# QuantumSavory/LDPCDecoders.jl

Measured on AMD Instinct MI355X. Metric: decoded syndromes/sec (batchdecode!, 50 iters) + achieved HBM GB/s fraction, higher is better.
Workload: dtype f64

## Files before the change

### ldpcdecoders.jl_amd/csrc/bp_kernels.hpp

```cpp
#pragma once
#include <hip/hip_runtime.h>
#include <stdint.h>

#include "team_layout.hpp"

namespace ldpc {

typedef unsigned long long u64;

#ifndef LDPC_MIN_WAVES
#define LDPC_MIN_WAVES 6
#endif
#ifndef LDPC_STM_SC1
#define LDPC_STM_SC1 0
#endif
#ifndef LDPC_NT
#define LDPC_NT 0
#endif
#ifndef LDPC_ROTATE
#define LDPC_ROTATE 1
#endif
#ifndef LDPC_PHASE_TICKS
#define LDPC_PHASE_TICKS 1
#endif
#ifndef LDPC_SLOT_PAD
#define LDPC_SLOT_PAD 1053184
#endif

template <int DC, int DV, int THREADS>
constexpr int min_waves_per_simd()
{
    constexpr int one_block = THREADS / 256;
#ifndef LDPC_MIN_WAVES_MID
#define LDPC_MIN_WAVES_MID 3
#endif
    int want = (DC <= 8 && DV <= 4) ? LDPC_MIN_WAVES : (DC <= 16 ? LDPC_MIN_WAVES_MID : 2);
    if (want < one_block) want = one_block;
    if (THREADS >= 1024 && want > 4) want = 4;
    return want;
}

#ifndef LDPC_LOADS_FIRST
#define LDPC_LOADS_FIRST 0
#endif
__device__ __forceinline__ void loads_first()
{
#if LDPC_LOADS_FIRST
    __builtin_amdgcn_sched_barrier(0);
#endif
}

__device__ __forceinline__ double ldm(const double *p)
{
#if LDPC_NT
    return __builtin_nontemporal_load(p);
#else
    return *p;
#endif
}
__device__ __forceinline__ void stm(double *p, double v)
{
#if LDPC_STM_SC1
    __hip_atomic_store(p, v, __ATOMIC_RELAXED, __HIP_MEMORY_SCOPE_AGENT);
#elif LDPC_NT
    __builtin_nontemporal_store(v, p);
#else
    *p = v;
#endif
}

struct BPCold {
    int *iters;
// ... 187 lines not shown
        out[k] = TF ? t : (1.0 - t) / (1.0 + t);
        S = S * a[k];
    }
#endif
}

template <int D, bool FIRST, bool TF = false>
__device__ __forceinline__ double check_update_exact(double *M, double sigma, double r, double S0 = 1.0)
{
    double a[D];
    if (FIRST) {
        const double a0 = 2.0 / (1.0 + r) - 1.0;
#pragma unroll
        for (int k = 0; k < D; ++k) a[k] = a0;
    } else {
        double m[D];
#pragma unroll
        for (int k = 0; k < D; ++k) m[k] = ldm(M + (size_t)k * kTile);
        check_factors<D>(m, a);
    }
    return check_finish_exact<D, TF>(M, a, sigma, S0);
}

template <int D, bool TF = false>
__device__ __forceinline__ void check_update_pair(double *M0, double *M1, double sigma0, double sigma1)
{
    double m0[D], m1[D];
#pragma unroll
    for (int k = 0; k < D; ++k) m0[k] = ldm(M0 + (size_t)k * kTile);
#pragma unroll
    for (int k = 0; k < D; ++k) m1[k] = ldm(M1 + (size_t)k * kTile);
    loads_first();
    double a[D];
    check_factors<D>(m0, a);
    check_finish_exact<D, TF>(M0, a, sigma0);
    check_factors<D>(m1, a);
    check_finish_exact<D, TF>(M1, a, sigma1);
}

template <bool FIRST>
__device__ __noinline__ void check_update_any(double *M, int deg, double sigma, double r)
{
    double S = 1.0;
    for (int k = deg - 1; k >= 0; --k) {
        double P = sigma;
        for (int q = 0; q < k; ++q) {
            const double m = FIRST ? r : M[(size_t)q * kTile];
            P = P * (2.0 / (1.0 + m) - 1.0);
        }
        const double mk = FIRST ? r : M[(size_t)k * kTile];
        const double ak = 2.0 / (1.0 + mk) - 1.0;
        const double t = P * S;
        M[(size_t)k * kTile] = (1.0 - t) / (1.0 + t);
        S = S * ak;
    }
// ... 180 lines not shown
    }
}

template <int DV>
__device__ __forceinline__ double bit_update(double *Mt, const int *__restrict__ pos, int deg, double r)
{
    if (deg == DV) return bit_update_exact<DV>(Mt, pos, r);
    if (deg == 0) return r;
    if (deg < DV) return bit_dispatch<1, DV - 1>(Mt, pos, deg, r);
    return bit_update_any(Mt, pos, deg, r);
}

__device__ __forceinline__ unsigned int defer_reserve(unsigned int *count, unsigned int cnt, unsigned int cap)
{
    unsigned int old = __hip_atomic_load(count, __ATOMIC_RELAXED, __HIP_MEMORY_SCOPE_AGENT);
    for (;;) {
        if (old + cnt > cap || old + cnt < old) return ~0u;
        const unsigned int prev = atomicCAS(count, old, old + cnt);
        if (prev == old) return old;
        old = prev;
    }
}

__device__ __forceinline__ void defer_copy_rows(const double *Mt, double *dst, bool mine, int nnz, int first, int step)
{
    int e = first;
    for (; e + 7 * step < nnz; e += 8 * step) {
        double v[8];
#pragma unroll
        for (int k = 0; k < 8; ++k) v[k] = Mt[(size_t)(e + k * step) * kTile];
        if (mine) {
#pragma unroll
            for (int k = 0; k < 8; ++k) dst[(size_t)(e + k * step) * kTile] = v[k];
        }
    }
    for (; e < nnz; e += step) {
        const double v = Mt[(size_t)e * kTile];
        if (mine) dst[(size_t)e * kTile] = v;
    }
}

template <int DC, int DV, bool WANT_LLR, int THREADS, bool SECOND>
__global__ void
__launch_bounds__(THREADS, (min_waves_per_simd<DC, DV, THREADS>()))
bp_tile_kernel(BPParams p, const int *__restrict__ row_ptr, const int *__restrict__ edge_bit,
               const int *__restrict__ col_ptr, const int *__restrict__ csc2csr,
               const u64 *__restrict__ synmask, const u64 *__restrict__ nevermask)
{
// ... 359 lines not shown
```

### ldpcdecoders.jl_amd/csrc/bp_team_kernels.hpp

```cpp
#pragma once
#include "bp_kernels.hpp"

#ifndef LDPC_TEAM_ROWS_WIDE
#define LDPC_TEAM_ROWS_WIDE 1
#endif
#ifndef LDPC_TEAM_TFORM
#define LDPC_TEAM_TFORM 1
#endif
#ifndef LDPC_TEAM_TEST_DIRECT
#define LDPC_TEAM_TEST_DIRECT 1
#endif
#ifndef LDPC_TEAM_SLEEP
#define LDPC_TEAM_SLEEP 16
#endif

namespace ldpc {


template <int DV>
struct TeamVRec {
    int pos[DV], lrow[DV], bit;
};
template <int DV>
__device__ __forceinline__ TeamVRec<DV> team_vrec_load(const int *__restrict__ vt)
// ... 203 lines not shown
                if ((polls & 31u) == 0u && wall_clock64() - t0 > (u64)ticks) {
                    bool dead = false;
                    while (c < (unsigned)G && !dead)
                        dead = __hip_atomic_compare_exchange_strong(word, &c, c | DEAD, __ATOMIC_RELAXED, __ATOMIC_RELAXED,
                                                                    __HIP_MEMORY_SCOPE_AGENT);
                    if (dead) __hip_atomic_store(fault, ticket | kTeamRollcallFailed, __ATOMIC_RELAXED, __HIP_MEMORY_SCOPE_SYSTEM);
                    if (dead || (c & DEAD)) { ok = 0; break; }
                }
            }
        }
        *sh_ok = ok;
    }
    __syncthreads();
    return *sh_ok != 0;
}

__device__ __forceinline__ int team_deal(unsigned int *counter, int lane)
{
    unsigned int t = 0;
    if (lane == 0) t = atomicAdd(counter, 1u);
    return __builtin_amdgcn_readfirstlane((int)t);
}

template <int D, bool FIRST, bool TF = false>
__device__ __forceinline__ void check_update_mixed(double *M, double *L, unsigned int mask, double sigma, double r)
{
    double *ptr[D];
    int nl = 0;
#pragma unroll
    for (int k = 0; k < D; ++k) {
        const bool in_lds = (mask >> k) & 1u;
        ptr[k] = in_lds ? L + (size_t)nl * kTile : M + (size_t)k * kTile;
        nl += in_lds ? 1 : 0;
    }
    double a[D], out[D];
    if (FIRST) {
        const double a0 = 2.0 / (1.0 + r) - 1.0;
#pragma unroll
        for (int k = 0; k < D; ++k) a[k] = a0;
    } else {
        double m[D];
#pragma unroll
        for (int k = 0; k < D; ++k) m[k] = *ptr[k];
        check_factors<D>(m, a);
    }
    check_compute_exact<D, TF>(a, sigma, out);
#pragma unroll
    for (int k = D - 1; k >= 0; --k) *ptr[k] = out[k];
}

template <int D, bool TF = false>
__device__ __forceinline__ double bit_update_mixed(double *Mt, double *L, const int (&pos)[D], const int (&lrow)[D], double r)
{
    double *ptr[D];
#pragma unroll
    for (int k = 0; k < D; ++k) {
        const bool in_lds = lrow[k] >= 0;
        ptr[k] = (in_lds ? L : Mt) + (size_t)(in_lds ? lrow[k] : pos[k]) * kTile;
    }
    double c[D], out[D];
#pragma unroll
    for (int k = 0; k < D; ++k) c[k] = *ptr[k];
    if (TF) check_to_odds<D>(c, c);
    const double F = bit_compute_exact<D>(c, r, out);
#pragma unroll
    for (int k = D - 1; k >= 0; --k) *ptr[k] = out[k];
    return F;
}

template <int D, bool FIRST, bool TF, class RGet, class RPut>
__device__ __forceinline__ void check_update_onchip(double *M, double *L, double *Ld, unsigned int mask, unsigned int rmask, int rbase,
                                                    double sigma, double r, RGet &&rget, RPut &&rput)
{
    double *ptr[D];
    int nl = 0;
#pragma unroll
    for (int k = 0; k < D; ++k) {
        const bool in_lds = (mask >> k) & 1u, in_reg = (rmask >> k) & 1u;
        ptr[k] = in_reg ? Ld : (in_lds ? L + (size_t)nl * kTile : M + (size_t)k * kTile);
        nl += in_lds ? 1 : 0;
    }
    double a[D], out[D];
    if (FIRST) {
        const double a0 = 2.0 / (1.0 + r) - 1.0;
#pragma unroll
        for (int k = 0; k < D; ++k) a[k] = a0;
    } else {
        double m[D];
#pragma unroll
        for (int k = 0; k < D; ++k) m[k] = *ptr[k];
#pragma unroll
        for (int k = 0; k < D; ++k)
            if ((rmask >> k) & 1u) m[k] = rget(rbase + __builtin_popcount(rmask & ((1u << k) - 1u)));
        check_factors<D>(m, a);
    }
    check_compute_exact<D, TF>(a, sigma, out);
#pragma unroll
    for (int k = D - 1; k >= 0; --k) *ptr[k] = out[k];
#pragma unroll
    for (int k = D - 1; k >= 0; --k) rput((rmask >> k) & 1u, rbase + __builtin_popcount(rmask & ((1u << k) - 1u)), out[k]);
}

template <int D, bool TF, class RGet, class RPut>
__device__ __forceinline__ double bit_update_onchip(double *Mt, double *L, double *Ld, const int (&pos)[D], const int (&loc)[D], double r,
                                                    RGet &&rget, RPut &&rput)
{
    double *ptr[D];
#pragma unroll
    for (int k = 0; k < D; ++k) {
        const bool in_lds = loc[k] >= 0;
        ptr[k] = loc[k] <= -2 ? Ld : (in_lds ? L : Mt) + (size_t)(in_lds ? loc[k] : pos[k]) * kTile;
    }
    double c[D], out[D];
#pragma unroll
    for (int k = 0; k < D; ++k) c[k] = *ptr[k];
#pragma unroll
    for (int k = 0; k < D; ++k)
        if (loc[k] <= -2) c[k] = rget(-2 - loc[k]);
    if (TF) check_to_odds<D>(c, c);
    const double F = bit_compute_exact<D>(c, r, out);
#pragma unroll
    for (int k = D - 1; k >= 0; --k) *ptr[k] = out[k];
#pragma unroll
    for (int k = D - 1; k >= 0; --k) rput(loc[k] <= -2, -2 - loc[k], out[k]);
    return F;
}

template <int D, bool FIRST, bool TF, class RGet, class RPut>
__device__ __forceinline__ void check_update_regs(int rbase, double sigma, double r, RGet &&rget, RPut &&rput)
{
    double a[D], out[D];
    if (FIRST) {
        const double a0 = 2.0 / (1.0 + r) - 1.0;
#pragma unroll
        for (int k = 0; k < D; ++k) a[k] = a0;
    } else {
        double m[D];
#pragma unroll
        for (int k = 0; k < D; ++k) m[k] = rget(rbase + k);
        check_factors<D>(m, a);
    }
    check_compute_exact<D, TF>(a, sigma, out);
#pragma unroll
    for (int k = D - 1; k >= 0; --k) rput(true, rbase + k, out[k]);
}

template <int D, bool TF, class RGet, class RPut>
__device__ __forceinline__ void bit_update_pair_first(double *Mt, double *L, const int (&pos0)[D], const int loc0, const int (&pos1)[D],
                                                      const int loc1, double r, RGet &&rget, RPut &&rput, double &T0, double &T1)
{
    double c0[D], c1[D], o0[D], o1[D];
    size_t at0[D], at1[D];
#pragma unroll
    for (int k = 0; k < D; ++k) { at0[k] = (size_t)pos0[k] * kTile; at1[k] = (size_t)pos1[k] * kTile; }
#pragma unroll
    for (int k = 1; k < D; ++k) c0[k] = ldm(Mt + at0[k]);
#pragma unroll
    for (int k = 1; k < D; ++k) c1[k] = ldm(Mt + at1[k]);
    if (loc0 == -1) c0[0] = ldm(Mt + at0[0]);
    else if (loc0 >= 0) c0[0] = L[(size_t)loc0 * kTile];
    else c0[0] = rget(-2 - loc0);
    if (loc1 == -1) c1[0] = ldm(Mt + at1[0]);
    else if (loc1 >= 0) c1[0] = L[(size_t)loc1 * kTile];
    else c1[0] = rget(-2 - loc1);
    loads_first();
    if (TF) { check_to_odds<D>(c0, c0); check_to_odds<D>(c1, c1); }
    T0 = bit_compute_exact<D>(c0, r, o0);
#pragma unroll
    for (int k = D - 1; k >= 1; --k) stm(Mt + at0[k], o0[k]);
    if (loc0 == -1) stm(Mt + at0[0], o0[0]);
    else if (loc0 >= 0) L[(size_t)loc0 * kTile] = o0[0];
    else rput(true, -2 - loc0, o0[0]);
    T1 = bit_compute_exact<D>(c1, r, o1);
#pragma unroll
    for (int k = D - 1; k >= 1; --k) stm(Mt + at1[k], o1[k]);
    if (loc1 == -1) stm(Mt + at1[0], o1[0]);
    else if (loc1 >= 0) L[(size_t)loc1 * kTile] = o1[0];
    else rput(true, -2 - loc1, o1[0]);
}

template <int D, int NB, bool TF, int KIND, class RGet, class RPut>
__device__ __forceinline__ void bit_update_multi_first(double *Mt, double *L, const int (&pos)[NB][D], const int (&loc)[NB], double r,
                                                       RGet &&rget, RPut &&rput, double (&T)[NB])
{
    double c[NB][D];
#pragma unroll
    for (int b = 0; b < NB; ++b) {
#pragma unroll
        for (int k = 1; k < D; ++k) c[b][k] = ldm(Mt + (size_t)pos[b][k] * kTile);
    }
#pragma unroll
    for (int b = 0; b < NB; ++b) {
        if (KIND == 1) c[b][0] = L[(size_t)loc[b] * kTile];
        else if (KIND == 2) c[b][0] = rget(-2 - loc[b]);
        else if (loc[b] == -1) c[b][0] = ldm(Mt + (size_t)pos[b][0] * kTile);
        else if (loc[b] >= 0) c[b][0] = L[(size_t)loc[b] * kTile];
        else c[b][0] = rget(-2 - loc[b]);
    }
    loads_first();
#pragma unroll
    for (int b = 0; b < NB; ++b) {
        if (TF) check_to_odds<D>(c[b], c[b]);
        double o[D];
        T[b] = bit_compute_exact<D>(c[b], r, o);
#pragma unroll
        for (int k = D - 1; k >= 1; --k) stm(Mt + (size_t)pos[b][k] * kTile, o[k]);
        if (KIND == 1) L[(size_t)loc[b] * kTile] = o[0];
        else if (KIND == 2) rput(true, -2 - loc[b], o[0]);
        else if (loc[b] == -1) stm(Mt + (size_t)pos[b][0] * kTile, o[0]);
        else if (loc[b] >= 0) L[(size_t)loc[b] * kTile] = o[0];
        else rput(true, -2 - loc[b], o[0]);
    }
}

template <int D, int DC, bool TF, class RPut>
__device__ __forceinline__ double bit_update_first(double *Mt, double *L, const double *first, const u64 *__restrict__ syn, int lane,
                                                   const int (&pos)[D], const int (&loc)[D], double r, RPut &&rput)
{
    double c[D], out[D];
#pragma unroll
    for (int k = 0; k < D; ++k) {
        const int i = pos[k] / DC, place = pos[k] - i * DC;
        const bool odd = (syn[i] >> lane) & 1ull;
        c[k] = first[(odd ? DC : 0) + place];
    }
    if (TF) check_to_odds<D>(c, c);
    const double F = bit_compute_exact<D>(c, r, out);
#pragma unroll
    for (int k = D - 1; k >= 0; --k) {
        if (loc[k] == -1) stm(Mt + (size_t)pos[k] * kTile, out[k]);
        else if (loc[k] >= 0) L[(size_t)loc[k] * kTile] = out[k];
        else rput(true, -2 - loc[k], out[k]);
    }
    return F;
}

#ifndef LDPC_TEAM_TEST_SPREAD
#define LDPC_TEAM_TEST_SPREAD 1
#endif
#ifndef LDPC_TEAM_FAULT_BLOCKS
#ifdef LDPC_EXPERIMENTS
#define LDPC_TEAM_FAULT_BLOCKS 1
#else
#define LDPC_TEAM_FAULT_BLOCKS 0
#endif
#endif
#ifndef LDPC_TEAM_LIKELY
#define LDPC_TEAM_LIKELY 1
#endif
#ifndef LDPC_TEAM_FUSE_FIRST
#define LDPC_TEAM_FUSE_FIRST 1
#endif
#ifndef LDPC_TEAM_FUSE_DC_MAX
#define LDPC_TEAM_FUSE_DC_MAX 10
// ... 52 lines not shown
__global__ void
__launch_bounds__(THREADS, (team_min_waves_per_simd<DC, DV, THREADS, LROWS || IRR>()))
bp_team_kernel(BPParams p, TeamParams tp, const int *__restrict__ row_ptr, const int *__restrict__ edge_bit,
               const int *__restrict__ col_ptr, const int *__restrict__ csc2csr,
               const u64 *__restrict__ synmask, const u64 *__restrict__ nevermask)
{
    static_assert(!(LROWS && RESUMED), "packed tiles are decoded where they lie, all rows in global memory");
    static_assert(RR == 0 || (LROWS && RR == kTeamRegRows), "rows in registers come on top of the rows in LDS");
    static_assert(!IRR || (!LROWS && !RESUMED && RR == 0), "irregular graphs: whole checks in LDS, fresh tiles");
    constexpr int RS = IRR ? 2 : 1;
    constexpr bool kTeamHints = (LDPC_TEAM_LIKELY != 0) && DC <= LDPC_TEAM_LIKELY_DC_MAX;
    constexpr bool TF = LROWS && (LDPC_TEAM_TFORM != 0) && DC <= 8;
    auto rget = [&](const int row) -> double {
        if constexpr (RR > 0) return team_reg_get(row);
        else return 0.0;
    };
    auto rput = [&](const bool on, const int row, const double v) {
        if constexpr (RR > 0) {
            if (on) team_reg_put(row, v);
        }
    };
    extern __shared__ double lds_rows[];
    double *const Lr = lds_rows + (threadIdx.x & 63);
    double *const Ldummy = Lr + (size_t)tp.rows.R * kTile;
    __shared__ int sh_ok;
    __shared__ unsigned int sh_deal[2];
#if !LDPC_TEAM_TEST_DIRECT
    __shared__ u64 sh_mism[THREADS / 64];
#endif
    const int lane = threadIdx.x & 63;
    const int w = __builtin_amdgcn_readfirstlane(threadIdx.x >> 6);
    constexpr int W = THREADS / 64;
    const int s = p.s, n = p.n;
    const double r = p.r;
    constexpr bool kFuseFirst = LROWS && (LDPC_TEAM_FUSE_FIRST != 0) && DC <= LDPC_TEAM_FUSE_DC_MAX;
    __shared__ double sh_first[kFuseFirst ? 2 * DC : 1];
    if constexpr (kFuseFirst) {
        if (threadIdx.x < 2) {
            const double a0 = 2.0 / (1.0 + p.r) - 1.0;
            double a[DC], out[DC];
#pragma unroll
            for (int k = 0; k < DC; ++k) a[k] = a0;
            check_compute_exact<DC, TF>(a, threadIdx.x ? -1.0 : 1.0, out);
#pragma unroll
            for (int k = 0; k < DC; ++k) sh_first[threadIdx.x * DC + k] = out[k];
        }
    }
// ... 42 lines not shown

    for (int tile = team; tile < ntiles;) {
    double *const Mt = p.msg + (size_t)(resumed ? tile : team) * (size_t)p.slot_stride + lane;
    u64 *const mw = tp.mism + (size_t)tile * (size_t)tp.mism_stride;
    const u64 *syn = synmask + (size_t)tile * s;
    u64 *em = p.errmask + (size_t)tile * n;
    u64 *fin = p.finmask + (size_t)tile * n;
    const long long b0 = (long long)tile * kTile;
    const long long left = batch - b0;
    u64 deferred = 0;
    const u64 valid = left >= kTile ? ~0ull : ((1ull << left) - 1ull);
    const u64 never = nevermask[tile];
    u64 active = valid;
    const int it0 = (resumed && ((valid >> lane) & 1ull)) ? cd->it0[b0 + lane] : 0;
    int my_iters = 0, my_conv = 0, it = 0;

    const bool can_run_ahead = !resumed && tp.errmask_alt != nullptr && tp.ahead_min > 0;
    u64 *const em_even = em, *const em_odd = can_run_ahead ? tp.errmask_alt + (size_t)tile * n : em;
    bool have_check = false;
    bool quiet = true;

    auto check_sweep = [&](const bool first, const int skip = 0) {
        const int nch = (s + kTeamCheckChunk - 1) / kTeamCheckChunk;
        auto chunk = [&](int c) {
            const int i1 = min(s, (c + 1) * kTeamCheckChunk);
            if constexpr (LROWS) {
                typedef int v4i __attribute__((ext_vector_type(4)));
                typedef int v8i __attribute__((ext_vector_type(8)));
                constexpr int FULL = (1 << DC) - 1;
                auto one = [&](double *const M, const v4i ct, const double sg) {
                    if (RR > 0 && ct.z == FULL) {
                        if (first) check_update_regs<DC, true, TF>(ct.w, sg, r, rget, rput);
                        else check_update_regs<DC, false, TF>(ct.w, sg, r, rget, rput);
                    } else if (ct.x == FULL) {
                        if (first) check_update_exact<DC, true, TF>(Lr + (size_t)ct.y * kTile, sg, r);
                        else check_update_exact<DC, false, TF>(Lr + (size_t)ct.y * kTile, sg, r);
                    } else if (RR > 0 && ct.z != 0) {
                        if (first) check_update_onchip<DC, true, TF>(M, Lr + (size_t)ct.y * kTile, Ldummy, (unsigned int)ct.x, (unsigned int)ct.z, ct.w, sg, r, rget, rput);
                        else check_update_onchip<DC, false, TF>(M, Lr + (size_t)ct.y * kTile, Ldummy, (unsigned int)ct.x, (unsigned int)ct.z, ct.w, sg, r, rget, rput);
                    } else if (first) {
                        check_update_mixed<DC, true, TF>(M, Lr + (size_t)ct.y * kTile, (unsigned int)ct.x, sg, r);
                    } else if (ct.x == 0) {
                        check_update_exact<DC, false, TF>(M, sg, r);
                    } else {
                        check_update_mixed<DC, false, TF>(M, Lr + (size_t)ct.y * kTile, (unsigned int)ct.x, sg, r);
                    }
                };
                const int i = c * kTeamCheckChunk;
                if (LDPC_HOT(kTeamCheckChunk == 2 && i + 2 == i1)) {
                    const v8i ct = *(const v8i *)(col_ptr + 4 * i);
                    const u64 s0 = syn[i], s1 = syn[i + 1];
                    const double sg0 = ((s0 >> lane) & 1ull) ? -1.0 : 1.0, sg1 = ((s1 >> lane) & 1ull) ? -1.0 : 1.0;
                    double *const M0 = Mt + (size_t)i * DC * kTile, *const M1 = M0 + (size_t)DC * kTile;
                    if ((ct.s0 | ct.s2 | ct.s4 | ct.s6) == 0 && !first && tp.pairs) {
                        check_update_pair<DC, TF>(M0, M1, sg0, sg1);
                    } else {
                        one(M0, v4i{ct.s0, ct.s1, ct.s2, ct.s3}, sg0);
                        one(M1, v4i{ct.s4, ct.s5, ct.s6, ct.s7}, sg1);
                    }
                    return;
                }
                for (int ii = i; ii < i1; ++ii) {
                    const v4i ct = *(const v4i *)(col_ptr + 4 * ii);
                    one(Mt + (size_t)ii * DC * kTile, ct, ((syn[ii] >> lane) & 1ull) ? -1.0 : 1.0);
                }
                return;
            }
            if constexpr (IRR) {
                for (int i = c * kTeamCheckChunk; i < i1; ++i) {
                    const int e0 = row_ptr[2 * i], lb = row_ptr[2 * i + 1];
                    const int deg = row_ptr[2 * i + 2] - e0;
                    const double sigma = ((syn[i] >> lane) & 1ull) ? -1.0 : 1.0;
                    double *const M = lb >= 0 ? Lr + (size_t)lb * kTile : Mt + (size_t)e0 * kTile;
                    if (first) check_update<DC, true, true>(M, deg, sigma, r);
                    else check_update<DC, false, true>(M, deg, sigma, r);
                }
                return;
            }
// ... 21 lines not shown
            const int lc = (mirror >= 0 && l < stat) ? mirror - l : l;
            if (!(LROWS && lc < skip * W)) chunk(lc * G + rank);
            l = !tp.dynamic ? l + W : (l + W < stat ? l + W : stat + team_deal(&sh_deal[0], lane));
        }
    };
    auto check_pre = [&](const int pre) {
        if constexpr (LROWS) {
            typedef int v4i __attribute__((ext_vector_type(4)));
            constexpr int FULL = (1 << DC) - 1;
            for (int k = 0; k < pre; ++k) {
                const int c = (w + k * W) * G + rank;
                for (int i = c * kTeamCheckChunk; i < (c + 1) * kTeamCheckChunk; ++i) {
                    const v4i ct = *(const v4i *)(col_ptr + 4 * i);
                    const double sg = ((syn[i] >> lane) & 1ull) ? -1.0 : 1.0;
                    if (RR > 0 && ct.z == FULL) check_update_regs<DC, false, TF>(ct.w, sg, r, rget, rput);
                    else check_update_exact<DC, false, TF>(Lr + (size_t)ct.y * kTile, sg, r);
                }
            }
        }
    };
    auto var_sweep = [&](const bool first = false) {
        const int vb = (one_xcd || LROWS || IRR) ? 4 : 16;
        const int nch = (n + vb - 1) / vb;
        const bool cap_on = WANT_LLR && (tp.llr_raw == 4 || tp.llr_raw == 5) && ((active >> lane) & 1ull);
        const size_t cap_rows = ((size_t)n + 3) & ~(size_t)3;
        unsigned int *const cap32 = (unsigned int *)p.llr + (size_t)tile * cap_rows * kTile;
        double *const cap64 = p.llr + (size_t)tile * cap_rows * kTile;
        auto cap_at = [&](int pos) { return ((size_t)(pos >> 2) * kTile + lane) * 4 + (size_t)(pos & 3); };
        auto capture1 = [&](int pos, double T) {
            if (!cap_on) return;
            if (tp.llr_raw == 4) cap32[cap_at(pos)] = llr_hi32(T);
            else cap64[cap_at(pos)] = T;
        };
        auto capture2 = [&](int pos, double T0, double T1) {
            if (!cap_on) return;
            typedef unsigned int v2u __attribute__((ext_vector_type(2)));
            typedef double v2d __attribute__((ext_vector_type(2)));
            if (tp.llr_raw == 4) *(v2u *)(cap32 + cap_at(pos)) = v2u{llr_hi32(T0), llr_hi32(T1)};
            else *(v2d *)(cap64 + cap_at(pos)) = v2d{T0, T1};
        };
        auto capture4 = [&](int pos, const double (&T)[4]) {
            if (!cap_on) return;
            typedef unsigned int v4u __attribute__((ext_vector_type(4)));
            typedef double v2d __attribute__((ext_vector_type(2)));
            if (tp.llr_raw == 4) *(v4u *)(cap32 + cap_at(pos)) = v4u{llr_hi32(T[0]), llr_hi32(T[1]), llr_hi32(T[2]), llr_hi32(T[3])};
            else { *(v2d *)(cap64 + cap_at(pos)) = v2d{T[0], T[1]}; *(v2d *)(cap64 + cap_at(pos) + 2) = v2d{T[2], T[3]}; }
// ... 22 lines not shown
                            T[1] = bit_update_first<DV, DC, TF>(Mt, Lr, sh_first, syn, lane, B.pos, B.lrow, r, rput);
                            T[2] = bit_update_first<DV, DC, TF>(Mt, Lr, sh_first, syn, lane, C.pos, C.lrow, r, rput);
                            T[3] = bit_update_first<DV, DC, TF>(Mt, Lr, sh_first, syn, lane, D.pos, D.lrow, r, rput);
                            decide(j, A.bit & 0x7fffffff, T[0], false);
                            decide(j + 1, B.bit & 0x7fffffff, T[1], false);
                            decide(j + 2, C.bit & 0x7fffffff, T[2], false);
                            decide(j + 3, D.bit & 0x7fffffff, T[3], false);
                            capture4(j, T);
                            return;
                        }
                        for (; j < j1; ++j) {
                            const TeamVRec<DV> A = team_vrec_load<DV>(csc2csr + (size_t)j * VT);
                            decide(j, A.bit & 0x7fffffff, bit_update_first<DV, DC, TF>(Mt, Lr, sh_first, syn, lane, A.pos, A.lrow, r, rput));
                        }
                        return;
                    }
                }
                auto single = [&](const TeamVRec<DV> &a, const int pa) {
                    if (a.bit >= 0) { decide(pa, a.bit, bit_update_exact_v<DV, TF>(Mt, a.pos, r)); return; }
                    if constexpr (RR > 0) {
                        int lo = a.lrow[0];
#pragma unroll
                        for (int k = 1; k < DV; ++k) lo = min(lo, a.lrow[k]);
                        if (lo <= -2) { decide(pa, a.bit & 0x7fffffff, bit_update_onchip<DV, TF>(Mt, Lr, Ldummy, a.pos, a.lrow, r, rget, rput)); return; }
                    }
                    decide(pa, a.bit & 0x7fffffff, bit_update_mixed<DV, TF>(Mt, Lr, a.pos, a.lrow, r));
                };
                auto two = [&](const TeamVRec<DV> &a, const TeamVRec<DV> &b, const int pa) {
                    int rest = -1;
#pragma unroll
                    for (int k = 1; k < DV; ++k) rest &= a.lrow[k] & b.lrow[k];
                    if ((a.bit | b.bit) >= 0 && tp.pairs) {
                        double T0, T1;
                        bit_update_pair_v<DV, TF>(Mt, a.pos, b.pos, r, T0, T1);
                        decide(pa, a.bit, T0, false);
                        decide(pa + 1, b.bit, T1, false);
                        capture2(pa, T0, T1);
                    } else if (rest == -1 && tp.pairs) {
                        double T0, T1;
                        bit_update_pair_first<DV, TF>(Mt, Lr, a.pos, a.lrow[0], b.pos, b.lrow[0], r, rget, rput, T0, T1);
                        decide(pa, a.bit & 0x7fffffff, T0, false);
                        decide(pa + 1, b.bit & 0x7fffffff, T1, false);
                        capture2(pa, T0, T1);
                    } else {
                        single(a, pa);
                        single(b, pa + 1);
                    }
// ... 171 lines not shown
                const int *const le = tp.rows.lds_edge + (size_t)rank * tp.rows.R;
                for (int q = w; q < tp.rows.R; q += W) {
                    const int e = le[q];
                    if (e >= 0) Mt[(size_t)e * kTile] = Lr[(size_t)q * kTile];
                }
                if constexpr (RR > 0) {
                    const int *const re = tp.rows.reg_edge + (size_t)(rank * W + w) * tp.rows.regs;
                    for (int q = 0; q < tp.rows.regs; ++q) {
                        const int e = __builtin_amdgcn_readfirstlane(re[q]);
                        if (e >= 0) Mt[(size_t)e * kTile] = rget(q);
                    }
                }
            }
            if (rank == 0 && threadIdx.x == 0)
                __hip_atomic_store(ctr + 33, defer_reserve(cd->defer_count, (unsigned)__popcll(active), cd->next_cap) + 1u,
                                   __ATOMIC_RELAXED, __HIP_MEMORY_SCOPE_AGENT);
            if (!team_barrier(ctr, G, rank, ++epoch, tp.fault, tp.ticket, &sh_ok, one_xcd, sh_deal)) return;
            const unsigned told = __hip_atomic_load(ctr + 33, __ATOMIC_RELAXED, __HIP_MEMORY_SCOPE_AGENT);
            if (!team_barrier(ctr, G, rank, ++epoch, tp.fault, tp.ticket, &sh_ok, one_xcd, sh_deal)) return;
            if (told != 0u) {
                const unsigned base = told - 1u;
                const bool mine = (active >> lane) & 1ull;
                const unsigned q = base + __builtin_amdgcn_mbcnt_hi((unsigned)(active >> 32), __builtin_amdgcn_mbcnt_lo((unsigned)active, 0u));
                defer_copy_rows(Mt, cd->next_state + (size_t)(q >> 6) * (size_t)cd->next_stride + (q & 63u), mine, p.nnz, gw, GW);
                if (rank == 0 && w == 0 && mine) {
                    cd->defer_list[q] = resumed ? cd->index[b0 + lane] : (int)(b0 + lane);
                    cd->defer_it[q] = total;
                }
                deferred = active;
                active = 0;
            }
        }
    }
    horizon = it;
    if (rank == 0 && w == 0) {
        if (((valid & ~deferred) >> lane) & 1ull) {
            const long long ob = resumed ? (long long)cd->index[b0 + lane] : b0 + lane;
            cd->conv[ob] = (unsigned char)my_conv;
            if (cd->iters) cd->iters[ob] = my_iters;
            tot_iters += my_iters;
        }
    }
    if (ntiles <= nteams) break;
    if (rank == 0 && threadIdx.x == 0)
        __hip_atomic_store(ctr + 34, (unsigned)nteams + __hip_atomic_fetch_add(tile_queue, 1u, __ATOMIC_RELAXED, __HIP_MEMORY_SCOPE_AGENT),
                           __ATOMIC_RELAXED, __HIP_MEMORY_SCOPE_AGENT);
    if (!team_barrier(ctr, G, rank, ++epoch, tp.fault, tp.ticket, &sh_ok, one_xcd, sh_deal)) return;
// ... 26 lines not shown
```

### ldpcdecoders.jl_amd/csrc/ldpc_mi355x.hip

```cpp
#include "../../include/ldpc_mi355x.h"
#include "../../include/ldpc_mi355x_debug.h"
#define LDPC_AUX_KERNELS 1
#include "bp_kernels.hpp"
#include "bp_lds_kernels.hpp"
#include "bp_node_kernels.hpp"
#include "bp_team_kernels.hpp"
#include "bit_io_kernels.hpp"
#include "pickers.hpp"
#include "team_plan.hpp"
#include "host_env.hpp"
#include "host_common.hpp"

#include <algorithm>
#include <atomic>
#include <cstdio>
#include <cstdlib>
#include <cstring>
#include <memory>
#include <mutex>
#include <new>
#include <string>
#include <thread>
#include <utility>
#include <vector>
// ... 1418 lines not shown
        if (plan.scatter && !d->team_ahead_set && tp.ahead_min > 0) tp.ahead_min = 1;
        team_kernel_t tk = pick_team_kernel(d->max_cdeg, d->max_bdeg, want_llr);
        size_t team_lds = team_lds_bytes();
        const int *t_col = a_col, *t_c2r = a_c2r, *t_row = a_row;
        if (plan.irr && !team_scatter && team_irr_build(d, team) == LDPC_OK && d->irr_on_chip > 0) {
            team_kernel_t tki = pick_team_kernel_irr(d->irr_dcb, d->max_bdeg, want_llr);
            const size_t need = (size_t)d->irr_R * kTile * sizeof(double);
            int occ_irr = 0;
            if (tki && d->prepare_kernel((const void *)tki, LDPC_TEAM_THREADS, need, &occ_irr) == LDPC_OK && occ_irr >= 1) {
                tk = tki; team_lds = need;
                d->last_lds_rows = d->irr_R; d->last_rows_on_chip = d->irr_on_chip;
                tp.rows.lds_edge = (const int *)d->irr_lds_edge.p;
                tp.rows.R = d->irr_R;
                tp.rows.reg_edge = nullptr; tp.rows.regs = 0;
                tp.rows.static_c = tp.rows.static_v = LDPC_TEAM_THREADS / 64; tp.rows.flip = 0;
                t_row = (const int *)d->irr_ctab.p;
                t_col = (const int *)d->irr_ptab.p;
                t_c2r = (const int *)d->irr_ploc.p;
                llr_posmap = (const int *)d->irr_posmap.p;
            }
        }
        if (plan.rows && team_rows_build(d, team) == LDPC_OK) {
            team_kernel_t tkr = pick_team_kernel_rows(d->rows_dc, d->rows_dv, want_llr, d->rows_regs > 0);
            const size_t need = (size_t)(d->rows_R + (d->rows_regs > 0 ? 1 : 0)) * kTile * sizeof(double);
            int occ_rows = 0;
            if (tkr && d->prepare_kernel((const void *)tkr, LDPC_TEAM_THREADS, need, &occ_rows) == LDPC_OK && occ_rows >= 1) {
                tk = tkr; team_lds = need;
                d->last_lds_rows = d->rows_R; d->last_rows_on_chip = d->rows_on_chip;
                tp.rows.lds_edge = (const int *)d->rows_lds_edge.p;
                tp.rows.R = d->rows_R;
                tp.rows.reg_edge = (const int *)d->rows_reg_edge.p;
                tp.rows.regs = d->rows_regs;
                tp.rows.static_c = d->rows_static_c; tp.rows.static_v = d->rows_static_v; tp.rows.flip = d->team_flip;
                tp.rows.first_c = d->rows_first_c;
                tp.pre = std::min((plan.wide && !d->team_pre_set) ? 8 : d->team_pre, d->rows_first_c / (LDPC_TEAM_THREADS / 64));
                t_col = (const int *)d->rows_ctab.p;
                t_c2r = (const int *)d->rows_vtab.p;
                llr_posmap = (const int *)d->rows_posmap.p;
            }
        }
        const u64 *a_syn = (const u64 *)d->synmask.p, *a_nev = (const u64 *)d->nevermask.p;
        void *args[] = {&p, &tp, &t_row, &a_eb, &t_col, &t_c2r, &a_syn, &a_nev};
        const hipError_t te = launch_team_grid(d, tk, team_grid, args, stream, team_lds);
        if (te != hipSuccess) {
            (void)hipGetLastError();
            d->team_max = 1;
            threads = tile_threads; grid = tile_grid;
// ... 610 lines not shown
```

Baseline: 94420.

## Split LDS and global message loads with address-space casts and branchless selects

Rewrites the mixed and on-chip check and bit updates in the team rows kernels into one template. Global and LDS operands are now loaded unconditionally through separate address-space-typed pointers and then selected, instead of going through generic pointers picked per edge. This lets the compiler emit ds_/global_ instructions and issue both load streams together. The change also removes the dummy LDS row, adds explicit waitcnt fences and scheduling barriers, and types the defer-copy destination as global. The cost is redundant dummy loads for edges that are not used, plus the risk that a hand-coded waitcnt conflicts with the compiler's own scheduling.

Measured after the change: 94560 (median of 5 runs). About the same (+0.1%).

```diff
diff --git a/ldpcdecoders.jl_amd/csrc/bp_kernels.hpp b/ldpcdecoders.jl_amd/csrc/bp_kernels.hpp
--- a/ldpcdecoders.jl_amd/csrc/bp_kernels.hpp
+++ b/ldpcdecoders.jl_amd/csrc/bp_kernels.hpp
@@ -43,11 +43,10 @@
 #ifndef LDPC_LOADS_FIRST
 #define LDPC_LOADS_FIRST 0
 #endif
+template <bool ON = (LDPC_LOADS_FIRST != 0)>
 __device__ __forceinline__ void loads_first()
 {
-#if LDPC_LOADS_FIRST
-    __builtin_amdgcn_sched_barrier(0);
-#endif
+    if constexpr (ON) __builtin_amdgcn_sched_barrier(0);
 }
 
 __device__ __forceinline__ double ldm(const double *p)
@@ -281,7 +280,7 @@
     return check_finish_exact<D, TF>(M, a, sigma, S0);
 }
 
-template <int D, bool TF = false>
+template <int D, bool TF = false, bool LF = (LDPC_LOADS_FIRST != 0)>
 __device__ __forceinline__ void check_update_pair(double *M0, double *M1, double sigma0, double sigma1)
 {
     double m0[D], m1[D];
@@ -289,7 +288,7 @@
     for (int k = 0; k < D; ++k) m0[k] = ldm(M0 + (size_t)k * kTile);
 #pragma unroll
     for (int k = 0; k < D; ++k) m1[k] = ldm(M1 + (size_t)k * kTile);
-    loads_first();
+    loads_first<LF>();
     double a[D];
     check_factors<D>(m0, a);
     check_finish_exact<D, TF>(M0, a, sigma0);
@@ -516,8 +515,11 @@
     }
 }
 
-__device__ __forceinline__ void defer_copy_rows(const double *Mt, double *dst, bool mine, int nnz, int first, int step)
-{
+template <bool GLOBAL_DST = false>
+__device__ __forceinline__ void defer_copy_rows(const double *Mt, double *dst_generic, bool mine, int nnz, int first, int step)
+{
+    typedef __attribute__((address_space(1))) double glb_f64;
+    typename std::conditional<GLOBAL_DST, glb_f64, double>::type *const dst = (decltype(dst))dst_generic;
     int e = first;
     for (; e + 7 * step < nnz; e += 8 * step) {
         double v[8];
diff --git a/ldpcdecoders.jl_amd/csrc/bp_team_kernels.hpp b/ldpcdecoders.jl_amd/csrc/bp_team_kernels.hpp
--- a/ldpcdecoders.jl_amd/csrc/bp_team_kernels.hpp
+++ b/ldpcdecoders.jl_amd/csrc/bp_team_kernels.hpp
@@ -249,64 +249,113 @@
     return __builtin_amdgcn_readfirstlane((int)t);
 }
 
-template <int D, bool FIRST, bool TF = false>
-__device__ __forceinline__ void check_update_mixed(double *M, double *L, unsigned int mask, double sigma, double r)
-{
-    double *ptr[D];
-    int nl = 0;
-#pragma unroll
-    for (int k = 0; k < D; ++k) {
-        const bool in_lds = (mask >> k) & 1u;
-        ptr[k] = in_lds ? L + (size_t)nl * kTile : M + (size_t)k * kTile;
-        nl += in_lds ? 1 : 0;
-    }
+__device__ __forceinline__ void team_counters_known() { __builtin_amdgcn_s_waitcnt(0x0070); }
+
+typedef __attribute__((address_space(3))) double lds_f64;
+
+template <int D, bool FIRST, bool TF, bool REGS, class RGet, class RPut>
+__device__ __forceinline__ void check_update_rows(double *M, double *L, double *Ld, unsigned int mask, unsigned int rmask, int rbase,
+                                                  double sigma, double r, RGet &&rget, RPut &&rput)
+{
+    lds_f64 *const Ll = (lds_f64 *)L, *const Lz = (lds_f64 *)Ld;
+    if (!REGS) rmask = 0u;
+    int lrow[D], nl = 0;
+#pragma unroll
+    for (int k = 0; k < D; ++k) { lrow[k] = nl; nl += (mask >> k) & 1u; }
     double a[D], out[D];
     if (FIRST) {
         const double a0 = 2.0 / (1.0 + r) - 1.0;
 #pragma unroll
         for (int k = 0; k < D; ++k) a[k] = a0;
     } else {
-        double m[D];
-#pragma unroll
-        for (int k = 0; k < D; ++k) m[k] = *ptr[k];
+        const int kz = min(D - 1, (int)__builtin_ctz(~(mask | rmask)));
+        double mg[D], ml[D], m[D];
+#pragma unroll
+        for (int k = 0; k < D; ++k) mg[k] = ldm(M + (size_t)((((mask | rmask) >> k) & 1u) ? kz : k) * kTile);
+#pragma unroll
+        for (int k = 0; k < D; ++k) ml[k] = ((mask >> k) & 1u) ? Ll[(size_t)lrow[k] * kTile] : *Lz;
+        team_counters_known();
+#pragma unroll
+        for (int k = 0; k < D; ++k) m[k] = ((mask >> k) & 1u) ? ml[k] : mg[k];
+        if constexpr (REGS) {
+#pragma unroll
+            for (int k = 0; k < D; ++k)
+                if ((rmask >> k) & 1u) m[k] = rget(rbase + __builtin_popcount(rmask & ((1u << k) - 1u)));
+        }
         check_factors<D>(m, a);
     }
     check_compute_exact<D, TF>(a, sigma, out);
 #pragma unroll
-    for (int k = D - 1; k >= 0; --k) *ptr[k] = out[k];
-}
-
-template <int D, bool TF = false>
-__device__ __forceinline__ double bit_update_mixed(double *Mt, double *L, const int (&pos)[D], const int (&lrow)[D], double r)
-{
-    double *ptr[D];
-#pragma unroll
-    for (int k = 0; k < D; ++k) {
-        const bool in_lds = lrow[k] >= 0;
-        ptr[k] = (in_lds ? L : Mt) + (size_t)(in_lds ? lrow[k] : pos[k]) * kTile;
-    }
-    double c[D], out[D];
-#pragma unroll
-    for (int k = 0; k < D; ++k) c[k] = *ptr[k];
-    if (TF) check_to_odds<D>(c, c);
-    const double F = bit_compute_exact<D>(c, r, out);
-#pragma unroll
-    for (int k = D - 1; k >= 0; --k) *ptr[k] = out[k];
-    return F;
-}
-
+    for (int k = D - 1; k >= 0; --k) {
+        if ((mask >> k) & 1u) Ll[(size_t)lrow[k] * kTile] = out[k];
+        else if (!((rmask >> k) & 1u)) stm(M + (size_t)k * kTile, out[k]);
+    }
+    if constexpr (REGS) {
+#pragma unroll
+        for (int k = D - 1; k >= 0; --k) rput((rmask >> k) & 1u, rbase + __builtin_popcount(rmask & ((1u << k) - 1u)), out[k]);
+    }
+}
+template <int D, bool FIRST, bool TF = false>
+__device__ __forceinline__ void check_update_mixed(double *M, double *L, double *Ld, unsigned int mask, double sigma, double r)
+{
+    check_update_rows<D, FIRST, TF, false>(M, L, Ld, mask, 0u, 0, sigma, r, [](int) { return 0.0; }, [](bool, int, double) {});
+}
 template <int D, bool FIRST, bool TF, class RGet, class RPut>
 __device__ __forceinline__ void check_update_onchip(double *M, double *L, double *Ld, unsigned int mask, unsigned int rmask, int rbase,
                                                     double sigma, double r, RGet &&rget, RPut &&rput)
 {
-    double *ptr[D];
-    int nl = 0;
-#pragma unroll
-    for (int k = 0; k < D; ++k) {
-        const bool in_lds = (mask >> k) & 1u, in_reg = (rmask >> k) & 1u;
-        ptr[k] = in_reg ? Ld : (in_lds ? L + (size_t)nl * kTile : M + (size_t)k * kTile);
-        nl += in_lds ? 1 : 0;
-    }
+    check_update_rows<D, FIRST, TF, true>(M, L, Ld, mask, rmask, rbase, sigma, r, rget, rput);
+}
+
+template <int D, bool TF, bool REGS, class RGet, class RPut>
+__device__ __forceinline__ double bit_update_rows(double *Mt, double *L, const int (&pos)[D], const int (&loc)[D], double r,
+                                                  RGet &&rget, RPut &&rput)
+{
+    lds_f64 *const Ll = (lds_f64 *)L;
+    int pz = pos[D - 1];
+#pragma unroll
+    for (int k = D - 2; k >= 0; --k) pz = loc[k] == -1 ? pos[k] : pz;
+    double cg[D], cl[D], c[D], out[D];
+#pragma unroll
+    for (int k = 0; k < D; ++k) cg[k] = ldm(Mt + (size_t)(loc[k] == -1 ? pos[k] : pz) * kTile);
+#pragma unroll
+    for (int k = 0; k < D; ++k) cl[k] = Ll[(size_t)(loc[k] >= 0 ? loc[k] : 0) * kTile];
+    team_counters_known();
+#pragma unroll
+    for (int k = 0; k < D; ++k) c[k] = loc[k] >= 0 ? cl[k] : cg[k];
+    if constexpr (REGS) {
+#pragma unroll
+        for (int k = 0; k < D; ++k)
+            if (loc[k] <= -2) c[k] = rget(-2 - loc[k]);
+    }
+    if (TF) check_to_odds<D>(c, c);
+    const double F = bit_compute_exact<D>(c, r, out);
+#pragma unroll
+    for (int k = D - 1; k >= 0; --k) {
+        if (loc[k] >= 0) Ll[(size_t)loc[k] * kTile] = out[k];
+        else if (loc[k] == -1) stm(Mt + (size_t)pos[k] * kTile, out[k]);
+    }
+    if constexpr (REGS) {
+#pragma unroll
+        for (int k = D - 1; k >= 0; --k) rput(loc[k] <= -2, -2 - loc[k], out[k]);
+    }
+    return F;
+}
+template <int D, bool TF = false>
+__device__ __forceinline__ double bit_update_mixed(double *Mt, double *L, const int (&pos)[D], const int (&lrow)[D], double r)
+{
+    return bit_update_rows<D, TF, false>(Mt, L, pos, lrow, r, [](int) { return 0.0; }, [](bool, int, double) {});
+}
+template <int D, bool TF, class RGet, class RPut>
+__device__ __forceinline__ double bit_update_onchip(double *Mt, double *L, const int (&pos)[D], const int (&loc)[D], double r,
+                                                    RGet &&rget, RPut &&rput)
+{
+    return bit_update_rows<D, TF, true>(Mt, L, pos, loc, r, rget, rput);
+}
+
+template <int D, bool FIRST, bool TF, class RGet, class RPut>
+__device__ __forceinline__ void check_update_regs(int rbase, double sigma, double r, RGet &&rget, RPut &&rput)
+{
     double a[D], out[D];
     if (FIRST) {
         const double a0 = 2.0 / (1.0 + r) - 1.0;
@@ -315,55 +364,6 @@
     } else {
         double m[D];
 #pragma unroll
-        for (int k = 0; k < D; ++k) m[k] = *ptr[k];
-#pragma unroll
-        for (int k = 0; k < D; ++k)
-            if ((rmask >> k) & 1u) m[k] = rget(rbase + __builtin_popcount(rmask & ((1u << k) - 1u)));
-        check_factors<D>(m, a);
-    }
-    check_compute_exact<D, TF>(a, sigma, out);
-#pragma unroll
-    for (int k = D - 1; k >= 0; --k) *ptr[k] = out[k];
-#pragma unroll
-    for (int k = D - 1; k >= 0; --k) rput((rmask >> k) & 1u, rbase + __builtin_popcount(rmask & ((1u << k) - 1u)), out[k]);
-}
-
-template <int D, bool TF, class RGet, class RPut>
-__device__ __forceinline__ double bit_update_onchip(double *Mt, double *L, double *Ld, const int (&pos)[D], const int (&loc)[D], double r,
-                                                    RGet &&rget, RPut &&rput)
-{
-    double *ptr[D];
-#pragma unroll
-    for (int k = 0; k < D; ++k) {
-        const bool in_lds = loc[k] >= 0;
-        ptr[k] = loc[k] <= -2 ? Ld : (in_lds ? L : Mt) + (size_t)(in_lds ? loc[k] : pos[k]) * kTile;
-    }
-    double c[D], out[D];
-#pragma unroll
-    for (int k = 0; k < D; ++k) c[k] = *ptr[k];
-#pragma unroll
-    for (int k = 0; k < D; ++k)
-        if (loc[k] <= -2) c[k] = rget(-2 - loc[k]);
-    if (TF) check_to_odds<D>(c, c);
-    const double F = bit_compute_exact<D>(c, r, out);
-#pragma unroll
-    for (int k = D - 1; k >= 0; --k) *ptr[k] = out[k];
-#pragma unroll
-    for (int k = D - 1; k >= 0; --k) rput(loc[k] <= -2, -2 - loc[k], out[k]);
-    return F;
-}
-
-template <int D, bool FIRST, bool TF, class RGet, class RPut>
-__device__ __forceinline__ void check_update_regs(int rbase, double sigma, double r, RGet &&rget, RPut &&rput)
-{
-    double a[D], out[D];
-    if (FIRST) {
-        const double a0 = 2.0 / (1.0 + r) - 1.0;
-#pragma unroll
-        for (int k = 0; k < D; ++k) a[k] = a0;
-    } else {
-        double m[D];
-#pragma unroll
         for (int k = 0; k < D; ++k) m[k] = rget(rbase + k);
         check_factors<D>(m, a);
     }
@@ -376,6 +376,7 @@
 __device__ __forceinline__ void bit_update_pair_first(double *Mt, double *L, const int (&pos0)[D], const int loc0, const int (&pos1)[D],
                                                       const int loc1, double r, RGet &&rget, RPut &&rput, double &T0, double &T1)
 {
+    lds_f64 *const Ll = (lds_f64 *)L;
     double c0[D], c1[D], o0[D], o1[D];
     size_t at0[D], at1[D];
 #pragma unroll
@@ -385,10 +386,10 @@
 #pragma unroll
     for (int k = 1; k < D; ++k) c1[k] = ldm(Mt + at1[k]);
     if (loc0 == -1) c0[0] = ldm(Mt + at0[0]);
-    else if (loc0 >= 0) c0[0] = L[(size_t)loc0 * kTile];
+    else if (loc0 >= 0) c0[0] = Ll[(size_t)loc0 * kTile];
     else c0[0] = rget(-2 - loc0);
     if (loc1 == -1) c1[0] = ldm(Mt + at1[0]);
-    else if (loc1 >= 0) c1[0] = L[(size_t)loc1 * kTile];
+    else if (loc1 >= 0) c1[0] = Ll[(size_t)loc1 * kTile];
     else c1[0] = rget(-2 - loc1);
     loads_first();
     if (TF) { check_to_odds<D>(c0, c0); check_to_odds<D>(c1, c1); }
@@ -396,13 +397,13 @@
 #pragma unroll
     for (int k = D - 1; k >= 1; --k) stm(Mt + at0[k], o0[k]);
     if (loc0 == -1) stm(Mt + at0[0], o0[0]);
-    else if (loc0 >= 0) L[(size_t)loc0 * kTile] = o0[0];
+    else if (loc0 >= 0) Ll[(size_t)loc0 * kTile] = o0[0];
     else rput(true, -2 - loc0, o0[0]);
     T1 = bit_compute_exact<D>(c1, r, o1);
 #pragma unroll
     for (int k = D - 1; k >= 1; --k) stm(Mt + at1[k], o1[k]);
     if (loc1 == -1) stm(Mt + at1[0], o1[0]);
-    else if (loc1 >= 0) L[(size_t)loc1 * kTile] = o1[0];
+    else if (loc1 >= 0) Ll[(size_t)loc1 * kTile] = o1[0];
     else rput(true, -2 - loc1, o1[0]);
 }
 
@@ -410,21 +411,22 @@
 __device__ __forceinline__ void bit_update_multi_first(double *Mt, double *L, const int (&pos)[NB][D], const int (&loc)[NB], double r,
                                                        RGet &&rget, RPut &&rput, double (&T)[NB])
 {
+    lds_f64 *const Ll = (lds_f64 *)L;
     double c[NB][D];
 #pragma unroll
     for (int b = 0; b < NB; ++b) {
-#pragma unroll
-        for (int k = 1; k < D; ++k) c[b][k] = ldm(Mt + (size_t)pos[b][k] * kTile);
-    }
-#pragma unroll
-    for (int b = 0; b < NB; ++b) {
-        if (KIND == 1) c[b][0] = L[(size_t)loc[b] * kTile];
+        if (KIND == 1) c[b][0] = Ll[(size_t)loc[b] * kTile];
         else if (KIND == 2) c[b][0] = rget(-2 - loc[b]);
         else if (loc[b] == -1) c[b][0] = ldm(Mt + (size_t)pos[b][0] * kTile);
-        else if (loc[b] >= 0) c[b][0] = L[(size_t)loc[b] * kTile];
+        else if (loc[b] >= 0) c[b][0] = Ll[(size_t)loc[b] * kTile];
         else c[b][0] = rget(-2 - loc[b]);
     }
-    loads_first();
+#pragma unroll
+    for (int b = 0; b < NB; ++b) {
+#pragma unroll
+        for (int k = 1; k < D; ++k) c[b][k] = ldm(Mt + (size_t)pos[b][k] * kTile);
+        loads_first<true>();
+    }
 #pragma unroll
     for (int b = 0; b < NB; ++b) {
         if (TF) check_to_odds<D>(c[b], c[b]);
@@ -432,10 +434,10 @@
         T[b] = bit_compute_exact<D>(c[b], r, o);
 #pragma unroll
         for (int k = D - 1; k >= 1; --k) stm(Mt + (size_t)pos[b][k] * kTile, o[k]);
-        if (KIND == 1) L[(size_t)loc[b] * kTile] = o[0];
+        if (KIND == 1) Ll[(size_t)loc[b] * kTile] = o[0];
         else if (KIND == 2) rput(true, -2 - loc[b], o[0]);
         else if (loc[b] == -1) stm(Mt + (size_t)pos[b][0] * kTile, o[0]);
-        else if (loc[b] >= 0) L[(size_t)loc[b] * kTile] = o[0];
+        else if (loc[b] >= 0) Ll[(size_t)loc[b] * kTile] = o[0];
         else rput(true, -2 - loc[b], o[0]);
     }
 }
@@ -444,6 +446,7 @@
 __device__ __forceinline__ double bit_update_first(double *Mt, double *L, const double *first, const u64 *__restrict__ syn, int lane,
                                                    const int (&pos)[D], const int (&loc)[D], double r, RPut &&rput)
 {
+    lds_f64 *const Ll = (lds_f64 *)L;
     double c[D], out[D];
 #pragma unroll
     for (int k = 0; k < D; ++k) {
@@ -456,7 +459,7 @@
 #pragma unroll
     for (int k = D - 1; k >= 0; --k) {
         if (loc[k] == -1) stm(Mt + (size_t)pos[k] * kTile, out[k]);
-        else if (loc[k] >= 0) L[(size_t)loc[k] * kTile] = out[k];
+        else if (loc[k] >= 0) Ll[(size_t)loc[k] * kTile] = out[k];
         else rput(true, -2 - loc[k], out[k]);
     }
     return F;
@@ -555,7 +558,6 @@
     };
     extern __shared__ double lds_rows[];
     double *const Lr = lds_rows + (threadIdx.x & 63);
-    double *const Ldummy = Lr + (size_t)tp.rows.R * kTile;
     __shared__ int sh_ok;
     __shared__ unsigned int sh_deal[2];
 #if !LDPC_TEAM_TEST_DIRECT
@@ -644,6 +646,7 @@
 
     auto check_sweep = [&](const bool first, const int skip = 0) {
         const int nch = (s + kTeamCheckChunk - 1) / kTeamCheckChunk;
+        if constexpr (LROWS) team_counters_known();
         auto chunk = [&](int c) {
             const int i1 = min(s, (c + 1) * kTeamCheckChunk);
             if constexpr (LROWS) {
@@ -658,14 +661,14 @@
                         if (first) check_update_exact<DC, true, TF>(Lr + (size_t)ct.y * kTile, sg, r);
                         else check_update_exact<DC, false, TF>(Lr + (size_t)ct.y * kTile, sg, r);
                     } else if (RR > 0 && ct.z != 0) {
-                        if (first) check_update_onchip<DC, true, TF>(M, Lr + (size_t)ct.y * kTile, Ldummy, (unsigned int)ct.x, (unsigned int)ct.z, ct.w, sg, r, rget, rput);
-                        else check_update_onchip<DC, false, TF>(M, Lr + (size_t)ct.y * kTile, Ldummy, (unsigned int)ct.x, (unsigned int)ct.z, ct.w, sg, r, rget, rput);
+                        if (first) check_update_onchip<DC, true, TF>(M, Lr + (size_t)ct.y * kTile, Lr, (unsigned int)ct.x, (unsigned int)ct.z, ct.w, sg, r, rget, rput);
+                        else check_update_onchip<DC, false, TF>(M, Lr + (size_t)ct.y * kTile, Lr, (unsigned int)ct.x, (unsigned int)ct.z, ct.w, sg, r, rget, rput);
                     } else if (first) {
-                        check_update_mixed<DC, true, TF>(M, Lr + (size_t)ct.y * kTile, (unsigned int)ct.x, sg, r);
+                        check_update_mixed<DC, true, TF>(M, Lr + (size_t)ct.y * kTile, Lr, (unsigned int)ct.x, sg, r);
                     } else if (ct.x == 0) {
                         check_update_exact<DC, false, TF>(M, sg, r);
                     } else {
-                        check_update_mixed<DC, false, TF>(M, Lr + (size_t)ct.y * kTile, (unsigned int)ct.x, sg, r);
+                        check_update_mixed<DC, false, TF>(M, Lr + (size_t)ct.y * kTile, Lr, (unsigned int)ct.x, sg, r);
                     }
                 };
                 const int i = c * kTeamCheckChunk;
@@ -675,7 +678,7 @@
                     const double sg0 = ((s0 >> lane) & 1ull) ? -1.0 : 1.0, sg1 = ((s1 >> lane) & 1ull) ? -1.0 : 1.0;
                     double *const M0 = Mt + (size_t)i * DC * kTile, *const M1 = M0 + (size_t)DC * kTile;
                     if ((ct.s0 | ct.s2 | ct.s4 | ct.s6) == 0 && !first && tp.pairs) {
-                        check_update_pair<DC, TF>(M0, M1, sg0, sg1);
+                        check_update_pair<DC, TF, true>(M0, M1, sg0, sg1);
                     } else {
                         one(M0, v4i{ct.s0, ct.s1, ct.s2, ct.s3}, sg0);
                         one(M1, v4i{ct.s4, ct.s5, ct.s6, ct.s7}, sg1);
@@ -743,6 +746,7 @@
     auto var_sweep = [&](const bool first = false) {
         const int vb = (one_xcd || LROWS || IRR) ? 4 : 16;
         const int nch = (n + vb - 1) / vb;
+        if constexpr (LROWS) team_counters_known();
         const bool cap_on = WANT_LLR && (tp.llr_raw == 4 || tp.llr_raw == 5) && ((active >> lane) & 1ull);
         const size_t cap_rows = ((size_t)n + 3) & ~(size_t)3;
         unsigned int *const cap32 = (unsigned int *)p.llr + (size_t)tile * cap_rows * kTile;
@@ -811,7 +815,7 @@
                         int lo = a.lrow[0];
 #pragma unroll
                         for (int k = 1; k < DV; ++k) lo = min(lo, a.lrow[k]);
-                        if (lo <= -2) { decide(pa, a.bit & 0x7fffffff, bit_update_onchip<DV, TF>(Mt, Lr, Ldummy, a.pos, a.lrow, r, rget, rput)); return; }
+                        if (lo <= -2) { decide(pa, a.bit & 0x7fffffff, bit_update_onchip<DV, TF>(Mt, Lr, a.pos, a.lrow, r, rget, rput)); return; }
                     }
                     decide(pa, a.bit & 0x7fffffff, bit_update_mixed<DV, TF>(Mt, Lr, a.pos, a.lrow, r));
                 };
@@ -1029,7 +1033,7 @@
                 const unsigned base = told - 1u;
                 const bool mine = (active >> lane) & 1ull;
                 const unsigned q = base + __builtin_amdgcn_mbcnt_hi((unsigned)(active >> 32), __builtin_amdgcn_mbcnt_lo((unsigned)active, 0u));
-                defer_copy_rows(Mt, cd->next_state + (size_t)(q >> 6) * (size_t)cd->next_stride + (q & 63u), mine, p.nnz, gw, GW);
+                defer_copy_rows<LROWS>(Mt, cd->next_state + (size_t)(q >> 6) * (size_t)cd->next_stride + (q & 63u), mine, p.nnz, gw, GW);
                 if (rank == 0 && w == 0 && mine) {
                     cd->defer_list[q] = resumed ? cd->index[b0 + lane] : (int)(b0 + lane);
                     cd->defer_it[q] = total;
diff --git a/ldpcdecoders.jl_amd/csrc/ldpc_mi355x.hip b/ldpcdecoders.jl_amd/csrc/ldpc_mi355x.hip
--- a/ldpcdecoders.jl_amd/csrc/ldpc_mi355x.hip
+++ b/ldpcdecoders.jl_amd/csrc/ldpc_mi355x.hip
@@ -1464,7 +1464,7 @@
         }
         if (plan.rows && team_rows_build(d, team) == LDPC_OK) {
             team_kernel_t tkr = pick_team_kernel_rows(d->rows_dc, d->rows_dv, want_llr, d->rows_regs > 0);
-            const size_t need = (size_t)(d->rows_R + (d->rows_regs > 0 ? 1 : 0)) * kTile * sizeof(double);
+            const size_t need = (size_t)d->rows_R * kTile * sizeof(double);
             int occ_rows = 0;
             if (tkr && d->prepare_kernel((const void *)tkr, LDPC_TEAM_THREADS, need, &occ_rows) == LDPC_OK && occ_rows >= 1) {
                 tk = tkr; team_lds = need;
```
